# tud-amr/semantic_dsp_map

Hardware: AMD Instinct MI355X
Metric: Mvoxels updated/sec (256^3 grid, 2M particles, VKITTI2 camera; whole hot-path frame) (higher is better)
Workload: dtype f32

## Files before the change

### semantic_dsp_map_amd/csrc/kernels.hip

```cpp
#include <algorithm>

#include <type_traits>

#include <hip/hip_ext.h>
#include "sdm_internal.h"
#include "sdm_scratch.h"

#pragma clang fp contract(off)

namespace sdm {

namespace {

constexpr int TPB = 256;

#ifdef SDM_AB_TIMERS
}
__device__ unsigned long long g_dbg[6][8192 * 4];
namespace {
#define DBG_T() wall_clock64()
#define DBG_PUTK(k, i, v) do { if (blockIdx.x < 8192) g_dbg[k][blockIdx.x * 4 + (i)] = (unsigned long long)(v); } while (0)
#define DBG_PUT(i, v) DBG_PUTK(0, i, v)
#define DBG_LANE0(k, i) do { if (threadIdx.x == 0 && threadIdx.y == 0) DBG_PUTK(k, i, DBG_T()); } while (0)
#else
// ... 1659 lines not shown
  for (int j = 0; j < VIS_J; ++j) {
    if (code[j] == 0xffffffffu || flg[j]) continue;
    if (imz[j] <= imd[j]) {
      st.vts[lvv[j]] = (uint16_t)f.gts;
      mark_tile(st, lvv[j], f.epoch);
    }
  }
  __syncthreads();
  DBG_LANE0(1, 2);
  const uint32_t nf = n_full;
  for (uint32_t k = threadIdx.x; k < nf; k += TPB) {
    const uint32_t c = full_list[k];
    const uint32_t g = g0 + (c >> 6);
    const int ax = ((wlo + (int)(g % nwx)) << 6) + (int)(c & 63u);
    const int ay = f.bb0[1] + (int)((g / nwx) % by);
    const int az = f.bb0[2] + (int)(g / ((uint32_t)nwx * by));
    visibility_voxel<S>(d, f, st, sc, depth_img, ax, ay, az);
  }
  DBG_LANE0(1, 3);
  }
}

__device__ __forceinline__ void sift_down(uint32_t *a, uint32_t start, uint32_t end) {
  uint32_t root = start;
  while (2 * root + 1 <= end) {
    uint32_t child = 2 * root + 1, sw = root;
    if (a[sw] < a[child]) sw = child;
    if (child + 1 <= end && a[sw] < a[child + 1]) sw = child + 1;
    if (sw == root) return;
    uint32_t t = a[root];
    a[root] = a[sw];
    a[sw] = t;
    root = sw;
  }
}

constexpr int A7_ROWS = 16;
constexpr int A7_ITEMS = 16;
constexpr uint32_t CK_LIGHT_MAX = 4;
enum : uint8_t { CK_DONE = 0, CK_LIGHT = 1, CK_HEAVY = 2 };

__device__ __forceinline__ void ck_store(const Filter &flt, const Scratch &sc, float *__restrict__ ck_out, int finish, int p,
                                         const sdm_labeled_point &o, float ck) {
  if (finish) {
    const float ckk = ck * flt.p_detect + flt.noise_number;
    sc.ck_kappa[p] = ckk;
    sc.pix4[p] = make_float4(o.x, o.y, o.z, ckk);
    sc.pixt[p] = (uint32_t)o.track_id | (1u << 16);
  } else {
    ck_out[p] = ck;
  }
}

constexpr int BR_TPB = 640;
constexpr int BR_WAVES = BR_TPB / 64;
constexpr int BR_MAXW = 1 << ROW_COL_BITS;
template <int PPT>
__global__ __launch_bounds__(BR_TPB) __attribute__((amdgpu_waves_per_eu(PPT <= 4 ? 5 : 4, PPT <= 4 ? 5 : 4))) void k_bin_rows(Dims d, State st, Scratch sc) {
  static_assert(PPT == 2 || PPT == 4 || PPT * BR_TPB >= BR_MAXW, "eight pixels per thread cover the widest image");
  __shared__ uint32_t pre[BR_MAXW + 1];
  __shared__ uint32_t wave_tot[BR_WAVES];
  __shared__ uint32_t s_base;
  const int r = blockIdx.x;
  DBG_LANE0(2, 0);
  if (r == (int)gridDim.x - 1 && threadIdx.x < 64) alias_compact_wave(st);
  const bool overflow = sc.cnt->overflow != 0;
  const int lane = threadIdx.x & 63, wid = threadIdx.x >> 6;
  const int W = d.W;
  uint32_t c[PPT];
  const int j0 = PPT * (int)threadIdx.x;
#pragma unroll
  for (int u = 0; u < PPT; ++u) c[u] = (!overflow && j0 + u < W) ? sc.bin_count[r * W + j0 + u] : 0u;
  uint32_t sub_n = 0;
  if (threadIdx.x < ROW_SUBS && !overflow) {
    sub_n = sc.row_cnt[(size_t)(r * ROW_SUBS + threadIdx.x) * ROW_CNT_STRIDE];
    if (sub_n > sc.row_cap) sub_n = sc.row_cap;
  }
  uint32_t inc = 0;
#pragma unroll
  for (int u = 0; u < PPT; ++u) inc += c[u];
  const uint32_t mine = inc;
#pragma unroll
  for (int off = 1; off < 64; off <<= 1) {
    const uint32_t t = __shfl_up(inc, off, 64);
    if (lane >= off) inc += t;
  }
  if (lane == 63) wave_tot[wid] = inc;
  __syncthreads();
  uint32_t before = 0, total = 0;
#pragma unroll
  for (int w = 0; w < BR_WAVES; ++w) {
    if (w < wid) before += wave_tot[w];
    total += wave_tot[w];
  }
  {
    uint32_t run = before + inc - mine;
#pragma unroll
    for (int u = 0; u < PPT; ++u) {
      if (j0 + u < W) pre[j0 + u] = run;
      run += c[u];
    }
  }
  if (threadIdx.x == 0) {
    pre[W] = total;
    s_base = total ? atomicAdd(&sc.cnt->n_vis, total) : 0u;
    if (total && (s_base > sc.cap_vis || total > sc.cap_vis - s_base)) {
      sc.cnt->overflow = 1;
      pre[W] = 0;
    }
  }
  uint32_t sub_ex[ROW_SUBS + 1];
  {
    uint32_t run = 0;
#pragma unroll
    for (int k = 0; k < ROW_SUBS; ++k) {
      sub_ex[k] = run;
      run += (uint32_t)__shfl(sub_n, k, 64);
    }
    sub_ex[ROW_SUBS] = run;
  }
  __shared__ uint32_t s_sub[ROW_SUBS + 1];
  if (threadIdx.x == 0) {
#pragma unroll
    for (int k = 0; k <= ROW_SUBS; ++k) s_sub[k] = sub_ex[k];
  }
  __syncthreads();
  const uint32_t base = s_base;
  uint32_t *__restrict__ bs = sc.bin_start + (size_t)r * (W + 1);
  const bool row_over = total != 0 && pre[W] == 0;
  {
    const int h = d.window_half;
#pragma unroll
    for (int u = 0; u < PPT; ++u) {
      const int j = j0 + u;
      if (j < W) {
        const uint32_t n = row_over ? 0u : pre[j + h + 1 > W ? W : j + h + 1] - pre[j - h < 0 ? 0 : j - h];
        sc.row_win[r * W + j] = (uint8_t)(n > 255u ? 255u : n);
      }
    }
  }
  for (int j = threadIdx.x; j <= W; j += BR_TPB) bs[j] = row_over ? 0u : base + pre[j];
  if (total == 0 || row_over) {
    DBG_LANE0(2, 1);
    return;
  }
  const uint32_t n_row = s_sub[ROW_SUBS];
  for (uint32_t g = threadIdx.x; g < n_row; g += BR_TPB) {
    int sub = 0;
#pragma unroll
    for (int k = 1; k < ROW_SUBS; ++k) sub += s_sub[k] <= g ? 1 : 0;
    const uint2 e = sc.row_list[(size_t)(r * ROW_SUBS + sub) * sc.row_cap + (g - s_sub[sub])];
    sc.bin_idx[base + pre[e.y & (uint32_t)(BR_MAXW - 1)] + (e.y >> ROW_COL_BITS)] = e.x;
  }
  __syncthreads();
  const size_t slot_base = (size_t)d.v_begin << d.p_n;
#pragma unroll
  for (int u = 0; u < PPT; ++u) {
    const uint32_t n = c[u];
    if (!n) continue;
    const uint32_t p = (uint32_t)(r * W + j0 + u);
    const uint32_t s = base + pre[j0 + u];
    uint32_t *a = sc.bin_idx + s;
    auto small_bin = [&](auto kk) {
      constexpr int K = decltype(kk)::value;
      uint32_t v[K];
#pragma unroll
      for (int i = 0; i < K; ++i) v[i] = (uint32_t)i < n ? a[i] : 0xffffffffu;
#pragma unroll
      for (int pass = 0; pass < K; ++pass)
#pragma unroll
        for (int i = pass & 1; i + 1 < K; i += 2) {
          const uint32_t lo = v[i] < v[i + 1] ? v[i] : v[i + 1], hi = v[i] < v[i + 1] ? v[i + 1] : v[i];
          v[i] = lo;
          v[i + 1] = hi;
        }
#pragma unroll
      for (int i0 = 0; i0 < K; i0 += 8) {
        if ((uint32_t)i0 >= n) break;
        float4 q[8];
        float w8[8];
        uint16_t t8[8];
#pragma unroll
        for (int i = 0; i < 8; ++i)
          if ((uint32_t)(i0 + i) < n) {
            const size_t li = (size_t)v[i0 + i] - slot_base;
            q[i] = st.pos4[li];
            q[i].w = __uint_as_float((uint32_t)st.forget[li]);
            const SlotRef sr = slot_ref_li(st, d.p_n, li);
            w8[i] = sr.w();
            t8[i] = sr.track();
          }
#pragma unroll
        for (int i = 0; i < 8; ++i)
          if ((uint32_t)(i0 + i) < n) {
            if (n > 1) a[i0 + i] = v[i0 + i];
            sc.vp4[s + i0 + i] = make_float4(q[i].x, q[i].y, q[i].z, w8[i]);
            sc.vtf[s + i0 + i] = (uint32_t)t8[i] | ((__float_as_uint(q[i].w) & 0xffu) << 16);
            sc.vpix[s + i0 + i] = p;
          }
      }
    };
    if (n <= 8) {
      small_bin(std::integral_constant<int, 8>{});
      continue;
    }
    if (n <= 16) {
      small_bin(std::integral_constant<int, 16>{});
      continue;
    }
    if (n > 1) {
      if (n <= 32) {
        for (uint32_t i = 1; i < n; ++i) {
          uint32_t x = a[i];
          uint32_t j = i;
          while (j > 0 && a[j - 1] > x) {
            a[j] = a[j - 1];
            --j;
          }
          a[j] = x;
        }
      } else {
        for (int start = (int)(n - 2) / 2; start >= 0; --start) sift_down(a, (uint32_t)start, n - 1);
        for (uint32_t end = n - 1; end > 0; --end) {
          uint32_t t = a[end];
          a[end] = a[0];
          a[0] = t;
          sift_down(a, 0, end - 1);
        }
      }
    }
    for (uint32_t i = 0; i < n; ++i) {
      const size_t li = (size_t)a[i] - slot_base;
      const float4 q = st.pos4[li];
      const SlotRef sr = slot_ref_li(st, d.p_n, li);
      sc.vp4[s + i] = make_float4(q.x, q.y, q.z, sr.w());
      sc.vtf[s + i] = (uint32_t)sr.track() | ((uint32_t)st.forget[li] << 16);
      sc.vpix[s + i] = p;
    }
  }
  DBG_LANE0(2, 1);
}

__global__ __launch_bounds__(TPB) void k_ck_classify(Dims d, Filter flt, Scratch sc, float *__restrict__ ck_out, int finish) {
  const uint32_t p = blockIdx.x * blockDim.x + threadIdx.x;
  const int W = d.W, H = d.H, h = d.window_half;
  const bool in_image = p < (uint32_t)(W * H);
  const bool overflow = sc.cnt->overflow != 0;
  sdm_labeled_point o;
  o.is_valid = 0;
  uint32_t total = 0;
  if (in_image) {
    o = load_point(sc.fa->cloud, p);
    const int i = (int)p / W;
    uint32_t rw[A7_ROWS];
#pragma unroll
    for (int r = 0; r < A7_ROWS; ++r) {
      const int ni = i + r - h;
      const bool ok = r <= 2 * h && ni >= 0 && ni < H;
      rw[r] = sc.row_win[(int)p + (ok ? (r - h) * W : 0)];
    }
    __builtin_amdgcn_sched_barrier(0);
#pragma unroll
    for (int r = 0; r < A7_ROWS; ++r) {
      const int ni = i + r - h;
      total += (r <= 2 * h && ni >= 0 && ni < H) ? rw[r] : 0u;
    }
  }
  uint8_t cls = CK_DONE;
  if (in_image && o.is_valid && total != 0 && !overflow) cls = total <= CK_LIGHT_MAX ? CK_LIGHT : CK_HEAVY;
  const unsigned long long hm = __ballot(cls == CK_HEAVY);
  if (hm) {
    const uint32_t lane = threadIdx.x & 63u;
    const uint32_t shard = blockIdx.x & (VIS_SHARDS - 1);
    uint32_t base = 0;
    if (lane == 0) base = atomicAdd(&sc.cnt->shard[shard].heavy, (uint32_t)__popcll(hm));
    base = (uint32_t)__shfl((int)base, 0, 64);
    if (cls == CK_HEAVY) sc.ck_heavy[shard * sc.cap_heavy + base + (uint32_t)__popcll(hm & ((1ull << lane) - 1ull))] = p;
  }
  if (!in_image) return;
  if (!finish) {
    sc.pix4[p] = make_float4(o.x, o.y, o.z, 0.f);
    sc.pixt[p] = o.is_valid ? ((uint32_t)o.track_id | (1u << 16)) : 0u;
  }
  if (!o.is_valid) {
    if (finish) sc.pixt[p] = 0;
  } else if (cls == CK_DONE) {
    ck_store(flt, sc, ck_out, finish, (int)p, o, 0.f);
  }
  sc.ck_class[p] = cls;
}


template <bool FAST>
__device__ __forceinline__ float ck_term(const Filter &flt, const float *__restrict__ pdf, const float4 pv, const uint32_t tf,
                                         const sdm_labeled_point &o, float rsig, bool &skip) {
  const uint16_t ptrack = (uint16_t)(tf & 0xffffu);
  skip = flt.independent && ptrack != o.track_id;
  const float fg = flt.forget[(tf >> 16) & 7];
  float gk = query_pdf_r<FAST>(pdf, pv.x, o.x, o.sigma, rsig) * query_pdf_r<FAST>(pdf, pv.y, o.y, o.sigma, rsig) *
             query_pdf_r<FAST>(pdf, pv.z, o.z, o.sigma, rsig);
  if (!flt.independent) {
    gk *= fg;
    if (ptrack != o.track_id) gk *= flt.id_transition;
  }
  return pv.w * gk;
}

__device__ __forceinline__ void ck_light_pixel(const Dims &d, const Filter &flt, const State &st, const Scratch &sc,
                                               float *__restrict__ ck_out, int finish, int p) {
  const bool mine = p < d.W * d.H && sc.ck_class[p] == CK_LIGHT;
  sdm_labeled_point o;
  uint32_t ss[A7_ROWS], ee[A7_ROWS];
  if (mine) {
    o = load_point(sc.fa->cloud, p);
    const int h = d.window_half;
    const int i = p / d.W, j = p - i * d.W;
    const int j0 = j - h < 0 ? 0 : j - h;
    const int j1 = j + h >= d.W ? d.W - 1 : j + h;
#pragma unroll
    for (int r = 0; r < A7_ROWS; ++r) {
      const int ni = i + r - h;
      ss[r] = ee[r] = 0;
      if (r <= 2 * h && ni >= 0 && ni < d.H) {
        ss[r] = sc.bin_start[ni * (d.W + 1) + j0];
        ee[r] = sc.bin_start[ni * (d.W + 1) + j1 + 1];
      }
    }
  }
  float ck = 0.f;
  const float *__restrict__ pdf = st.pdf;
  const float rsig = mine ? div_recip(o.sigma) : 1.f;
  auto rows = [&](auto fast) {
#pragma unroll
    for (int r = 0; r < A7_ROWS; ++r) {
      if (ss[r] == ee[r]) continue;
      float acc = 0.f;
      for (uint32_t k = ss[r]; k < ee[r]; ++k) {
        bool skip;
        const float t = ck_term<decltype(fast)::value>(flt, pdf, sc.vp4[k], sc.vtf[k], o, rsig, skip);
        if (!skip) acc += t;
      }
      ck += acc;
    }
  };
  if (__ballot(rsig == 0.f) == 0ull) {
    if (mine) rows(std::true_type{});
  } else {
    if (mine) rows(std::false_type{});
  }
  if (mine) ck_store(flt, sc, ck_out, finish, p, o, ck);
}

#ifndef SDM_CK_TERM_CAP
#define SDM_CK_TERM_CAP 3584
#endif
constexpr uint32_t CK_TERM_CAP = SDM_CK_TERM_CAP;

#ifndef SDM_CK_HEAVY_PER_LIST
#define SDM_CK_HEAVY_PER_LIST 28
#endif
constexpr uint32_t CK_HEAVY_BLOCKS = SDM_CK_HEAVY_PER_LIST * VIS_SHARDS;
#ifndef SDM_CK_WAVES
#define SDM_CK_WAVES 7
#endif
#define CK_WAVES_ATTR __attribute__((amdgpu_waves_per_eu(SDM_CK_WAVES, SDM_CK_WAVES)))

__global__ __launch_bounds__(A7_ROWS *A7_ITEMS) CK_WAVES_ATTR void k_ck(Dims d, Filter flt, State st, Scratch sc,
                                                          float *__restrict__ ck_out, int finish) {
  DBG_LANE0(3, 0);
  if (blockIdx.x >= CK_HEAVY_BLOCKS) {
    ck_light_pixel(d, flt, st, sc, ck_out, finish,
                   (int)((blockIdx.x - CK_HEAVY_BLOCKS) * (A7_ROWS * A7_ITEMS) + threadIdx.y * A7_ROWS + threadIdx.x));
    DBG_LANE0(3, 1);
    return;
  }
  __shared__ float rowsum[A7_ITEMS][A7_ROWS];
  __shared__ uint32_t rowoff[A7_ITEMS * A7_ROWS + 1];
  __shared__ uint32_t rowbeg[A7_ITEMS * A7_ROWS];
  __shared__ float opx[A7_ITEMS][5];
  __shared__ uint32_t otrk[A7_ITEMS];
  __shared__ float term[CK_TERM_CAP];
  __shared__ uint8_t rowof[CK_TERM_CAP];
  const int r = threadIdx.x, it = threadIdx.y;
  const int lane = it * A7_ROWS + r;
  const int h = d.window_half;
  const uint32_t shard = blockIdx.x & (VIS_SHARDS - 1);
  const uint32_t n = sc.cnt->shard[shard].heavy;
  const float *__restrict__ pdf = st.pdf;
  const gptr<sdm_labeled_point> cloud_img = as_global(sc.fa->cloud);
  __shared__ uint32_t s_q0, s_slow;
  for (;;) {
    __syncthreads();
    if (lane == 0) {
      s_q0 = atomicAdd(&sc.cnt->shard[shard].heavy_ticket, (uint32_t)A7_ITEMS);
      s_slow = 0;
    }
    __syncthreads();
    const uint32_t q0 = s_q0;
    if (q0 >= n) break;
#ifdef SDM_AB_TIMERS
    if (lane == 0) g_dbg[3][blockIdx.x * 4 + 2] += 1;
#endif
    const uint32_t q = q0 + it;
    int p = 0;
    uint32_t s = 0, e = 0;
    sdm_labeled_point o;
    if (q < n) {
      p = (int)sc.ck_heavy[shard * sc.cap_heavy + q];
      o = load_point(sc.fa->cloud, p);
      const int i = p / d.W, j = p - i * d.W;
      const int ni = i + r - h;
      if (r <= 2 * h && ni >= 0 && ni < d.H) {
        const int j0 = j - h < 0 ? 0 : j - h;
        const int j1 = j + h >= d.W ? d.W - 1 : j + h;
        s = sc.bin_start[ni * (d.W + 1) + j0];
        e = sc.bin_start[ni * (d.W + 1) + j1 + 1];
      }
      if (r == 0) {
        opx[it][0] = o.x;
        opx[it][1] = o.y;
        opx[it][2] = o.z;
        opx[it][3] = o.sigma;
        opx[it][4] = div_recip(o.sigma);
        if (opx[it][4] == 0.f) s_slow = 1;
        otrk[it] = o.track_id;
// ... 1146 lines not shown
      SDM_DISPATCH_S(k_occupancy_scan_lists, sgrid, s, d, flt.occ_threshold, st, cnt, st.occ_need, grid.x, remark);
      SDM_DISPATCH_S(k_occupancy_listed, dim3(OCC_LISTED_GRID), s, d, flt.occ_threshold, st, remark);
    } else {
      SDM_DISPATCH_S(k_occupancy_scan, sgrid, s, d, flt.occ_threshold, st, cnt, st.occ_need, grid.x, remark);
    }
    SDM_DISPATCH_S(k_occupancy_dense, grid, s, d, flt.occ_threshold, st, cnt, st.occ_need, remark, grid.x);
  } else {
    const uint32_t n_tiles = grid.x;
    const uint32_t seg = n_tiles <= TPB * OCC_SEG_MAX ? ((n_tiles + TPB - 1) / TPB + 15u) / 16u * 16u : 0u;
    if (seg) grid = dim3(std::min<uint32_t>(OCC_GRID, n_tiles));
    SDM_DISPATCH_S(k_occupancy, grid, s, d, flt.occ_threshold, st, cnt, fa, n_tiles, seg);
  }
}


void launch_set_frame(FrameArgs *fa_dev, const FrameArgs &fa, hipStream_t s) {
  hipLaunchKernelGGL(k_set_frame, dim3(1), dim3(TPB), 0, s, fa_dev, fa);
}
const void *set_frame_kernel() { return reinterpret_cast<const void *>(k_set_frame); }

void launch_frustum(const Dims &d, const Scratch &sc, hipStream_t s) {
  static bool lds_attr_set = false;
  if (!lds_attr_set) {
    (void)hipFuncSetAttribute(reinterpret_cast<const void *>(k_flood2d), hipFuncAttributeMaxDynamicSharedMemorySize, 152 * 1024);
    lds_attr_set = true;
  }
  const size_t max_words = (size_t)(d.NY + 1) * (d.NZ + 1) * sc.wpl;
  const unsigned g_mask = (unsigned)std::min<size_t>(blocks_for(max_words * 64), 4096);
  const unsigned g_line = (unsigned)std::min<size_t>(blocks_for((size_t)sc.wy * (d.NZ + 1) * 64), 256);
  hipLaunchKernelGGL(k_vertex_mask, dim3(g_mask), dim3(TPB), 0, s, d, sc.fa_side, sc.vmask, sc.wpl, sc.cnt);
  hipLaunchKernelGGL(k_line_info, dim3(g_line), dim3(TPB), 0, s, d, sc.fa_side, sc.vmask, sc.wpl, sc.wy, sc.line_ne, sc.line_ey, sc.line_ez,
                     sc.cnt);
  hipLaunchKernelGGL(k_flood2d, dim3(1), dim3(TPB), (size_t)(d.NZ + 1) * sc.wy * 8 * 4, s, d, sc.fa_side, sc.vmask, sc.wpl, sc.wy, sc.line_ey,
                     sc.line_ez, sc.line_reach, sc.cnt);
  hipLaunchKernelGGL(k_flood_generic, dim3(1), dim3(1024), 0, s, d, sc.fa_side, sc.vmask, sc.reach, sc.wpl, sc.cnt);
}

void launch_visibility(const Dims &d, const Filter &flt, const State &st, const Scratch &sc, float *ck_out, int finish, hipStream_t s,
                       hipEvent_t vis_done) {
  {
    const size_t max_words = (size_t)((d.NX + 63) / 64 + 1) * d.NY * d.NZ;
    dim3 grid((unsigned)std::min<size_t>(blocks_for(max_words, VIS_WORDS), 2048));
    if (vis_done) {
      switch (d.p_n) {
        case 1: hipExtLaunchKernelGGL(k_visibility<2>, grid, dim3(TPB), 0, s, nullptr, vis_done, 0, d, st, sc); break;
        case 2: hipExtLaunchKernelGGL(k_visibility<4>, grid, dim3(TPB), 0, s, nullptr, vis_done, 0, d, st, sc); break;
        case 3: hipExtLaunchKernelGGL(k_visibility<8>, grid, dim3(TPB), 0, s, nullptr, vis_done, 0, d, st, sc); break;
        default: hipExtLaunchKernelGGL(k_visibility<16>, grid, dim3(TPB), 0, s, nullptr, vis_done, 0, d, st, sc); break;
      }
    } else {
      SDM_DISPATCH_S(k_visibility, grid, s, d, st, sc);
    }
  }
  if (d.W <= 2 * BR_TPB) hipLaunchKernelGGL(k_bin_rows<2>, dim3((unsigned)d.H), dim3(BR_TPB), 0, s, d, st, sc);
  else if (d.W <= 4 * BR_TPB) hipLaunchKernelGGL(k_bin_rows<4>, dim3((unsigned)d.H), dim3(BR_TPB), 0, s, d, st, sc);
  else hipLaunchKernelGGL(k_bin_rows<8>, dim3((unsigned)d.H), dim3(BR_TPB), 0, s, d, st, sc);
  hipLaunchKernelGGL(k_ck_classify, dim3(blocks_for((size_t)d.W * d.H)), dim3(TPB), 0, s, d, flt, sc, ck_out, finish);
}

void launch_ck(const Dims &d, const Filter &flt, const State &st, const Scratch &sc, float *ck_out, int finish, hipStream_t s) {
  hipLaunchKernelGGL(k_ck, dim3(CK_HEAVY_BLOCKS + blocks_for((size_t)d.W * d.H, A7_ROWS * A7_ITEMS)), dim3(A7_ROWS, A7_ITEMS), 0, s, d, flt, st, sc,
                     ck_out, finish);
}
void launch_ck_finish(const Dims &d, const Filter &flt, const Scratch &sc, const float *parts, int n_parts, size_t part_stride, hipStream_t s) {
  hipLaunchKernelGGL(k_ck_finish, dim3(blocks_for((size_t)d.W * d.H)), dim3(TPB), 0, s, d, flt, sc, parts, n_parts,
                     part_stride ? part_stride : (size_t)d.W * d.H);
}
void launch_ck_reduce_chunk(const float *stage, const float *own_part, float *full, uint32_t chunk, int world, int rank, hipStream_t s) {
  hipLaunchKernelGGL(k_ck_reduce_chunk, dim3((chunk + TPB - 1) / TPB), dim3(TPB), 0, s, stage, own_part, full, chunk, world, rank);
}
void launch_weight(const Dims &d, const Filter &flt, const State &st, const Scratch &sc, hipStream_t s, const float *ck_raw) {
  const int side = 2 * d.window_half + 1;
#define SDM_WEIGHT(UU, RR)                                                                                              \
  if (ck_raw) hipLaunchKernelGGL((k_weight<UU, RR, true>), dim3(WT_GRID), dim3(64 * WT_WAVES), 0, s, d, flt, st, sc, ck_raw); \
  else hipLaunchKernelGGL((k_weight<UU, RR, false>), dim3(WT_GRID), dim3(64 * WT_WAVES), 0, s, d, flt, st, sc, ck_raw);
  if (side * side <= 64) {
    SDM_WEIGHT(4, 1)
  } else if (side * side <= 128) {
    SDM_WEIGHT(4, 2)
  } else {
    SDM_WEIGHT(2, 4)
  }
#undef SDM_WEIGHT
}

int launch_birth_prepare(const Dims &d, const Filter &flt, const BirthOrder &bo, const State &st,
                         const Scratch &sc, hipStream_t s) {
  const size_t hw = (size_t)d.W * d.H;
  const size_t total = hw * flt.nb;
  if (flt.use_rng) {
    hipLaunchKernelGGL(k_birth_flags, dim3(blocks_for(hw)), dim3(TPB), 0, s, d, bo, sc);
    exclusive_scan_u32(sc.b_valid, sc.b_rank, hw, sc.scan_scratch_b, s);
  }
  hipLaunchKernelGGL(k_birth_candidates, dim3(blocks_for(total)), dim3(TPB), 0, s, d, flt, bo, st, sc);
  if (flt.use_rng) hipLaunchKernelGGL(k_birth_cursor, dim3(1), dim3(64), 0, s, d, flt, sc);
  int nbits = d.x_n + d.y_n + d.z_n + 1;
  return radix_sort_pairs(sc.bkey_a, sc.bval_a, sc.bkey_b, sc.bval_b, total, nbits, sc.sort_scratch, s);
}

void launch_birth_replay(const Dims &d, const Filter &flt, const State &st, const Scratch &sc, int which, bool literal,
                         hipStream_t s) {
  const size_t total = (size_t)d.W * d.H * flt.nb;
  const uint32_t *skey = which ? sc.bkey_b : sc.bkey_a;
  const uint32_t *sval = which ? sc.bval_b : sc.bval_a;
  dim3 grid(blocks_for(total));
#define SDM_BIRTH(SS)                                                                                                  \
  if (literal) hipLaunchKernelGGL((k_birth_replay<SS, true>), grid, dim3(TPB), 0, s, d, flt, st, sc, skey, sval, (uint32_t)total); \
  else hipLaunchKernelGGL((k_birth_replay<SS, false>), grid, dim3(TPB), 0, s, d, flt, st, sc, skey, sval, (uint32_t)total);
  switch (d.p_n) {
    case 1: SDM_BIRTH(2) break;
    case 2: SDM_BIRTH(4) break;
    case 3: SDM_BIRTH(8) break;
    default: SDM_BIRTH(16) break;
  }
#undef SDM_BIRTH
// ... 164 lines not shown
```

### semantic_dsp_map_amd/csrc/lifecycle.hip

```cpp
#include <rocrand/rocrand.h>

#include <chrono>
#include <cmath>
#include <cstdlib>
#include <mutex>

#include "sdm_map.h"

#pragma clang fp contract(off)

namespace {

thread_local std::string g_last_error;

__attribute__((constructor(101))) void sdm_runtime_defaults() {
  setenv("HIP_FORCE_DEV_KERNARG", "1", 0);
}

constexpr double GRAPH_PIECES_US = 110.0, GRAPH_CHAIN_US = 170.0;
constexpr int LAUNCHES_PER_FRAME = 50;

__global__ void k_noop() {}

}
// ... 390 lines not shown
  A(m->st.forget, n_slots);
  HIP_TRY(hipMemsetAsync(m->st.forget, 0, n_slots, m->stream));
  A(m->st.rec, rec_array_bytes(d.v_count, d.S));
  const size_t v_groups = ((size_t)d.v_count + 511) / 512 * 512;
  A(m->st.vts, v_groups + 64);
  A(m->st.vflag, v_groups + 64);
  m->st.tile_stride = (uint32_t)tile_mark_bytes(d);
  A(m->st.tile_dirty, 2 * (size_t)m->st.tile_stride);
  A(m->st.occ_need, ((size_t)d.v_count + 63) / 64 + 32);
  A(m->st.occ_list, occ_list_tiles(d.v_count) * OCC_LIST_CAP);
  A(m->st.occ_list_n, occ_list_tiles(d.v_count) + 64);
  m->st.occ_unit_cap = (uint32_t)((occ_list_tiles(d.v_count) + OCC_LIST_SHARDS - 1) / OCC_LIST_SHARDS * (OCC_LIST_CAP / OCC_LIST_UNIT));
  A(m->st.occ_unit, (size_t)OCC_LIST_SHARDS * m->st.occ_unit_cap);
  A(m->st.occ_shard, OCC_LIST_SHARDS + 1);
  HIP_TRY(hipMemsetAsync(m->st.occ_shard, 0, (OCC_LIST_SHARDS + 1) * sizeof(State::OccListShard), m->stream));
  A(m->st.grp_hint, grp_hint_bytes(d.v_count));
  HIP_TRY(hipMemsetAsync(m->st.grp_hint, 0, grp_hint_bytes(d.v_count), m->stream));
  A(m->st.owner, n_slots);
  A(m->st.owner_flag, owner_flag_bytes(n_slots));
  A(m->st.owner_flag2, owner_flag2_bytes(n_slots));
  A(m->st.alias, 2 + 2 * ALIAS_CAP);
  m->st.alias_cap = ALIAS_CAP;
  HIP_TRY(hipMemsetAsync(m->st.alias, 0, 8, m->stream));
  A(m->st.alias_filter, ALIAS_FILTER_WORDS);
  HIP_TRY(hipMemsetAsync(m->st.alias_filter, 0, ALIAS_FILTER_WORDS * 4, m->stream));
  A(m->st.res, d.v_count);
  A(m->st.stamps_x, d.NX);
  A(m->st.stamps_y, d.NY);
  A(m->st.stamps_z, d.NZ);
  A(m->st.pdf, PDF_NUM);
  m->noise_n = 1000000;
  A(m->st.noise, m->noise_n);
  HIP_TRY(hipMemsetAsync(m->st.noise, 0, (size_t)m->noise_n * 4, m->stream));
  {
    std::vector<float> pdf;
    build_pdf_table(pdf);
    HIP_TRY(hipMemcpyAsync(m->st.pdf, pdf.data(), PDF_NUM * 4, hipMemcpyHostToDevice, m->stream));
    HIP_TRY(hipStreamSynchronize(m->stream));
  }
  Scratch &sc = m->sc;
  sc.wpl = (int)((d.NX + 1 + 63) / 64);
  const size_t n_words = (size_t)(d.NZ + 1) * (d.NY + 1) * sc.wpl;
  A(sc.vmask, n_words);
  A(sc.reach, n_words);
  sc.wy = (int)((d.NY + 1 + 63) / 64);
  const size_t n_line_words = (size_t)(d.NZ + 1) * sc.wy;
  A(sc.line_ne, n_line_words);
  A(sc.line_ey, n_line_words);
  A(sc.line_ez, n_line_words);
  A(sc.line_reach, n_line_words);
  A(m->d_depth, hw);
  A(m->d_cloud, hw);
  A(sc.bin_count, hw + 1 + (size_t)d.H * ROW_SUBS * ROW_CNT_STRIDE);
  A(sc.row_win, hw);
  sc.row_cnt = sc.bin_count + hw + 1;
  A(sc.bin_start, (size_t)d.H * (d.W + 1));
  size_t cap_vis = cfg->max_visible > 0 ? (size_t)cfg->max_visible
                                        : std::min<size_t>(n_slots + (size_t)VIS_SHARDS * 256 * d.S, (size_t)16 << 20);
  cap_vis = (cap_vis + VIS_SHARDS - 1) / VIS_SHARDS * VIS_SHARDS;
  cap_vis = std::min<size_t>(cap_vis, 0xffffff00u);
  sc.cap_vis = (uint32_t)cap_vis;
  {
    const size_t row_total = std::min<size_t>(cap_vis, std::max<size_t>(2 * cap_vis / (size_t)d.H, (size_t)2 * d.W * d.S));
    sc.row_cap = (uint32_t)std::max<size_t>(64, (row_total + row_total / 4) / ROW_SUBS + 64);
  }
  A(sc.row_list, (size_t)d.H * ROW_SUBS * sc.row_cap);
  A(sc.bin_idx, cap_vis);
  A(sc.vpix, cap_vis);
  A(sc.vp4, cap_vis);
  A(sc.vtf, cap_vis);
  A(sc.pix4, hw);
  A(sc.pixt, hw);
  A(sc.ck_kappa, hw);
  sc.cap_heavy = (uint32_t)(((hw + 255) / 256 + VIS_SHARDS - 1) / VIS_SHARDS * 256);
  A(sc.ck_heavy, (size_t)sc.cap_heavy * VIS_SHARDS);
  A(sc.ck_class, hw);
  m->ck_chunk = (uint32_t)(((hw + shard_count - 1) / shard_count + 63) / 64 * 64);
  A(m->d_ck_part, (size_t)m->ck_chunk * shard_count);
  for (auto &r : m->raw) {
    A(r.depth, hw);
    A(r.static_mask, hw);
    A(r.label_to_inst, 256);
    A(r.bbox, 6 * MAX_CLOUD_OBJECTS);
  }
  A(sc.b_valid, hw + 1);
  A(sc.b_rank, hw + 1);
  sc.cap_move = (uint32_t)std::min<size_t>((size_t)d.V * d.S, (size_t)1 << 18);
  A(m->d_counts_local, HALO_OBJ);
  const size_t mv_cnt_n = move_count_elems();
  A(sc.mv_cnt, mv_cnt_n);
  A(sc.mv_list, 8192);
  A(sc.mv_nlist, 4);
  HIP_TRY(hipMemsetAsync(sc.mv_nlist, 0, 4 * sizeof(uint32_t), m->stream));
  A(sc.mv_nmem, 8192);
  A(sc.mv_mem, move_member_elems(n_slots));
  A(sc.mv_tot, move_total_elems());
  HIP_TRY(hipMemsetAsync(sc.mv_tot, 0, move_total_elems() * sizeof(uint32_t), m->stream));
  A(m->d_track_bits, 2048);
  A(sc.mv_copy, sc.cap_move);
  A(sc.track_to_obj, 65536);
  HIP_TRY(hipMemsetAsync(sc.track_to_obj, 0xFF, 65536, m->stream));
  size_t scan_need = scan_scratch_elems(hw + 1);
  A(sc.scan_scratch, scan_need + 16);
  A(sc.scan_scratch_b, scan_scratch_elems(hw + 1) + 16);
  HIP_TRY(hipMemsetAsync(sc.scan_scratch, 0, (scan_need + 16) * 4, m->stream));
  HIP_TRY(hipMemsetAsync(sc.scan_scratch_b, 0, (scan_scratch_elems(hw + 1) + 16) * 4, m->stream));
  A(sc.mv_row, (size_t)d.v_count * MV_ROW);
  HIP_TRY(hipMemsetAsync(sc.mv_row, 0xff, (size_t)d.v_count * MV_ROW * sizeof(uint32_t), m->stream));
  A(sc.mv_next, sc.cap_move);
  A(sc.cnt, 1);
  A(sc.cur, 1);
  HIP_TRY(hipMemsetAsync(sc.cnt, 0, sizeof(Counters), m->stream));
  HIP_TRY(hipMemsetAsync(sc.cur, 0, sizeof(Cursors), m->stream));
  A(m->d_fa[0], 1);
  A(m->d_fa[1], 1);
  A(m->d_fa[2], 1);
  for (FrameArgs *p : m->d_fa) HIP_TRY(hipMemsetAsync(p, 0, sizeof(FrameArgs), m->stream));
  m->sc.fa = m->d_fa[0];
  m->sc.fa_side = m->d_fa[1];
  m->sc.fa_moves = m->d_fa[2];
  A(m->d_u64, 1);
  A(m->emit.mask, emit_mask_bytes(d));
  A(m->emit.blk_cnt, emit_block_elems(d));
  A(m->emit.total, 4);
#undef A
  m->cur_depth = m->d_depth;
  m->cur_cloud = m->d_cloud;
  {
    const char *e = getenv("SDM_GRAPH");
// ... 181 lines not shown
```

### semantic_dsp_map_amd/csrc/sdm_internal.h

```cpp
#pragma once
#include <hip/hip_runtime.h>
#include <stdint.h>

#include "../../include/sdm.h"

#pragma clang fp contract(off)

namespace sdm {

constexpr uint32_t INVALID_INDEX = 0xffffffffu;
constexpr uint16_t OWNER_NONE = 0xFFFF;
constexpr int PDF_NUM = 20000;
#define SDM_OCC_INIT_WEIGHT 0.05f
#define SDM_MIN_RIGHT_PDF 0.1f

enum : uint8_t { ST_INVALID = 0, ST_UPDATED = 1, ST_REGULAR_BORN = 2, ST_GUESSED_BORN = 3, ST_COPIED = 4, ST_TIMEPTC = 5 };

struct Dims {
  int x_n, y_n, z_n, p_n;
  uint32_t NX, NY, NZ, S;
  uint32_t V;
  uint32_t v_begin;
  uint32_t v_count;
  uint32_t rz_begin, rz_count;
// ... 4 lines not shown
  float dmin, dmax;
  float tanx, tany;
  float occl_coeff;
  int window_half;
  int max_movable;
};

struct Frame {
  int eq[3];
  float center[3];
  uint32_t gts;
  uint32_t epoch;
  float E[16];
  int bb0[3], bb1[3];
  int start_v[3];
  int start_ok;
};

struct Filter {
  float p_detect, noise_number, occ_threshold, id_transition;
  float forget[8];
  int independent;
  int consider_depth_noise;
  int nb;
  int use_rng;
  int noise_n;
};

struct Counters {
  uint32_t n_vis;
  uint32_t n_birth_success;
  uint32_t n_birth_attempts;
  uint32_t n_resampled;
  uint32_t n_moved;
  uint32_t n_move_reinserted;
  uint32_t n_frustum_voxels;
  uint32_t n_occupied;
  uint32_t n_free;
  uint32_t overflow;
  uint32_t n_valid_px;
  uint32_t n_halo_dropped;
  uint32_t vis_flood_complex, vis_flood_rounds, vis_start_in_frustum;
  uint32_t n_moved_b[2];
  uint32_t pad[2];
  struct alignas(128) ShardLine {
    uint32_t vis;
    uint32_t fv;
    uint32_t heavy;
    uint32_t birth;
    uint32_t resample;
    uint32_t sweep;
    uint32_t sweep_tiles;
    uint32_t heavy_ticket;
    uint32_t pad[24];
  };
  ShardLine shard[64];
  uint32_t flood_complex;
  uint32_t flood_rounds;
  uint32_t start_in_frustum;
  uint32_t flood_pad[29];
};
static_assert(sizeof(Counters::ShardLine) == 128, "one cache line per shard");
constexpr uint32_t VIS_SHARDS = 64;
constexpr uint32_t ROW_SUBS = 8;
constexpr int ROW_COL_BITS = 12, ROW_PIB_BITS = 32 - ROW_COL_BITS;
constexpr uint32_t ROW_CNT_STRIDE = 32;
constexpr uint32_t OWNER_CHUNK = 4096;
constexpr uint32_t OWNER_GROUP = 64;
__host__ __device__ constexpr size_t owner_flag_bytes(size_t n_slots) {
  return ((n_slots + OWNER_CHUNK - 1) / OWNER_CHUNK + OWNER_GROUP - 1) / OWNER_GROUP * OWNER_GROUP;
}
__host__ __device__ constexpr size_t owner_flag2_bytes(size_t n_slots) { return (owner_flag_bytes(n_slots) / OWNER_GROUP + 4095) / 4096 * 4096; }
constexpr int MAX_STAMP_UPDATES = 96;
struct StampUpdates {
  int n;
  uint32_t value;
  uint16_t entry[MAX_STAMP_UPDATES];
};
struct Cursors {
  int32_t birth_cursor;
  int32_t move_cursor;
  uint32_t move_list_overflow;
};

constexpr size_t REC_BYTES_PER_SLOT = 10;
__host__ __device__ constexpr uint32_t rec_bytes(uint32_t S) { return (uint32_t)REC_BYTES_PER_SLOT * (S - 1u); }
__host__ __device__ constexpr size_t rec_array_bytes(size_t v_count, uint32_t S) { return (v_count + 64) * rec_bytes(S) + 64; }
typedef float rec_f32 __attribute__((aligned(2)));
typedef uint32_t rec_v4u __attribute__((ext_vector_type(4), aligned(2)));
typedef uint32_t rec_v2u __attribute__((ext_vector_type(2), aligned(2)));

struct SlotRef {
  unsigned char *r;
  uint32_t L, k;
  __host__ __device__ __forceinline__ float w() const { return *reinterpret_cast<const rec_f32 *>(r + 4u * k); }
  __host__ __device__ __forceinline__ uint16_t ts() const { return *reinterpret_cast<const uint16_t *>(r + 4u * L + 2u * k); }
  __host__ __device__ __forceinline__ uint16_t track() const { return *reinterpret_cast<const uint16_t *>(r + 6u * L + 2u * k); }
  __host__ __device__ __forceinline__ uint8_t label() const { return r[8u * L + k]; }
  __host__ __device__ __forceinline__ uint8_t status() const { return r[9u * L + k]; }
  __host__ __device__ __forceinline__ void set_w(float v) const { *reinterpret_cast<rec_f32 *>(r + 4u * k) = v; }
  __host__ __device__ __forceinline__ void set_ts(uint16_t v) const { *reinterpret_cast<uint16_t *>(r + 4u * L + 2u * k) = v; }
  __host__ __device__ __forceinline__ void set_track(uint16_t v) const { *reinterpret_cast<uint16_t *>(r + 6u * L + 2u * k) = v; }
  __host__ __device__ __forceinline__ void set_label(uint8_t v) const { r[8u * L + k] = v; }
  __host__ __device__ __forceinline__ void set_status(uint8_t v) const { r[9u * L + k] = v; }
};

struct State {
  float4 *pos4 = nullptr;
  uint8_t *forget = nullptr;
  unsigned char *rec = nullptr;
  uint16_t *vts = nullptr;
  uint8_t *vflag = nullptr;
  uint8_t *tile_dirty = nullptr;
  uint32_t tile_stride = 0;
  unsigned long long *occ_need = nullptr;
  uint16_t *occ_list = nullptr;
  uint32_t *occ_list_n = nullptr;
  uint2 *occ_unit = nullptr;
  uint32_t occ_unit_cap = 0;
// ... 353 lines not shown
```

### semantic_dsp_map_amd/csrc/sdm_scratch.h

```cpp
#pragma once
#include "sdm_internal.h"

namespace sdm {

struct BirthOrder {
  int off[10];
  int cols[9];
};

struct MoveCopy {
  float x, y, z;
  uint32_t forget_bits;
  float w;
  uint16_t ts, track, owner;
  uint8_t label, status;
  uint32_t voxel;
};
static_assert(sizeof(MoveCopy) == 32, "MoveCopy layout");

constexpr int MAX_MOVE_OBJECTS = 48;
constexpr int MAX_REMOVE_TRACKS = 128;
constexpr int HALO_OBJ = 64;
constexpr int HALO_RECORD_BYTES = 36;
constexpr int HALO_HEADER_BYTES = 16;
__host__ __device__ constexpr size_t halo_segment_bytes(uint32_t cap) { return HALO_HEADER_BYTES + (size_t)cap * HALO_RECORD_BYTES; }
struct MoveSet {
  int n;
  float T[MAX_MOVE_OBJECTS][12];
  uint16_t track[MAX_MOVE_OBJECTS];
};

struct FrameArgs {
  Frame f;
  StampUpdates su;
  MoveSet ms;
  int n_obj;
  int n_remove;
  uint32_t mv_seq;
  uint32_t mv_batch;
  int force_generic;
  const float *depth;
  const sdm_labeled_point *cloud;
  uint16_t remove[MAX_REMOVE_TRACKS];
};
static_assert(sizeof(FrameArgs) <= 3400, "FrameArgs travels as a kernel argument (4 KB limit, with the launch's other arguments)");

constexpr int MV_ROW = 16;
constexpr int MV_DIRECT = MV_ROW - 2;
constexpr uint32_t MV_FIRST = 0x100u;
struct Scratch {
  const FrameArgs *fa = nullptr;
  const FrameArgs *fa_side = nullptr;
  const FrameArgs *fa_moves = nullptr;
  uint64_t *vmask = nullptr, *reach = nullptr;
  int wpl = 0;
  uint64_t *line_ne = nullptr, *line_ey = nullptr, *line_ez = nullptr, *line_reach = nullptr;
  int wy = 0;
  uint32_t *bin_count = nullptr, *bin_start = nullptr;
  uint32_t *row_cnt = nullptr;
  uint8_t *row_win = nullptr;
  uint2 *row_list = nullptr;
  uint32_t row_cap = 0;
  uint32_t cap_vis = 0;
  uint32_t *bin_idx = nullptr, *vpix = nullptr;
  float4 *vp4 = nullptr;
  uint32_t *vtf = nullptr;
  float4 *pix4 = nullptr;
  uint32_t *pixt = nullptr;
  float *ck_kappa = nullptr;
  uint8_t *ck_class = nullptr;
  uint32_t *ck_heavy = nullptr;
  uint32_t cap_heavy = 0;
  uint32_t *b_valid = nullptr, *b_rank = nullptr;
  uint32_t *bkey_a = nullptr, *bval_a = nullptr, *bkey_b = nullptr, *bval_b = nullptr;
  float4 *bpos = nullptr;
  uint32_t *mv_cnt = nullptr;
  uint32_t *mv_list = nullptr, *mv_nlist = nullptr;
  uint32_t *mv_nmem = nullptr, *mv_mem = nullptr, *mv_tot = nullptr;
  MoveCopy *mv_copy = nullptr;
  uint32_t cap_move = 0;
  unsigned char *halo_send = nullptr;
  const unsigned char *halo_recv = nullptr;
  uint32_t halo_cap = 0;
  uint32_t halo_world = 1;
  uint8_t *track_to_obj = nullptr;
  uint32_t *scan_scratch = nullptr, *sort_scratch = nullptr;
  uint32_t *scan_scratch_b = nullptr;
  uint32_t *mv_row = nullptr, *mv_next = nullptr;
  Counters *cnt = nullptr;
  Cursors *cur = nullptr;
};

constexpr int MAX_CLOUD_OBJECTS = 64;
struct CloudArgsHost {
  double R[9], t[3];
  double ifx, icx, ify, icy;
  double dmin, dmax;
  float sigma0, sigma1;
  int consider_depth_noise, consider_instance, n_objects, has_static;
  int sky_instance, has_bbox;
  int track[MAX_CLOUD_OBJECTS], label[MAX_CLOUD_OBJECTS];
};
void launch_labeled_cloud(const Dims &d, const CloudArgsHost &h, const float *depth, const uint8_t *static_mask,
                          const uint16_t *label_to_inst, const uint8_t *obj_masks, const double *bbox,
                          sdm_labeled_point *cloud, hipStream_t s);
void launch_manual_resize(const Dims &d, const void *src, void *dst, int src_w, int src_h, float scale, int elem_bytes,
                          hipStream_t s);

void launch_set_frame(FrameArgs *fa_dev, const FrameArgs &fa, hipStream_t s);
const void *set_frame_kernel();
struct MembersArgs {
  uint32_t *mv_cnt, *mv_list, *mv_nlist, *mv_nmem, *mv_mem, *mv_tot;
  Cursors *cur;
  uint32_t n_flags;
  size_t n_slots;
};
struct FrameBeginLaunch {
#ifndef SDM_FB_GRID
#define SDM_FB_GRID 1024
#endif
  static constexpr unsigned GRID = SDM_FB_GRID, BLOCK = 256;
  Counters *cnt;
  uint32_t *bin_count;
  uint32_t n_bins;
// ... 71 lines not shown
```

Before: 95850.

## Fuse pixel classification into row binning and compact light pixels into lists

Moves the per-pixel light/heavy classification, previously its own kernel reading a row_win byte plane, into k_bin_rows. That kernel now reads bin_count over the vertical window, forms column sums in shared memory and sums them horizontally. Light pixels are now compacted into sharded lists like heavy ones, so the ck kernel launches a fixed grid that walks those lists instead of one block per image tile checking a class byte. This removes a kernel launch, the row_win and ck_class buffers and idle light blocks. In exchange k_bin_rows does more loads and register work per thread, and the output order of the lists changes.

```diff
diff --git a/semantic_dsp_map_amd/csrc/kernels.hip b/semantic_dsp_map_amd/csrc/kernels.hip
--- a/semantic_dsp_map_amd/csrc/kernels.hip
+++ b/semantic_dsp_map_amd/csrc/kernels.hip
@@ -1735,30 +1735,66 @@
   }
 }
 
-constexpr int BR_TPB = 640;
-constexpr int BR_WAVES = BR_TPB / 64;
 constexpr int BR_MAXW = 1 << ROW_COL_BITS;
 template <int PPT>
-__global__ __launch_bounds__(BR_TPB) __attribute__((amdgpu_waves_per_eu(PPT <= 4 ? 5 : 4, PPT <= 4 ? 5 : 4))) void k_bin_rows(Dims d, State st, Scratch sc) {
+__global__ __launch_bounds__(BR_TPB) __attribute__((amdgpu_waves_per_eu(PPT <= 4 ? 5 : 4, PPT <= 4 ? 5 : 4))) void k_bin_rows(
+    Dims d, Filter flt, State st, Scratch sc, float *__restrict__ ck_out, int finish) {
   static_assert(PPT == 2 || PPT == 4 || PPT * BR_TPB >= BR_MAXW, "eight pixels per thread cover the widest image");
   __shared__ uint32_t pre[BR_MAXW + 1];
+  __shared__ uint32_t colsum[BR_MAXW];
   __shared__ uint32_t wave_tot[BR_WAVES];
   __shared__ uint32_t s_base;
   const int r = blockIdx.x;
   DBG_LANE0(2, 0);
   if (r == (int)gridDim.x - 1 && threadIdx.x < 64) alias_compact_wave(st);
-  const bool overflow = sc.cnt->overflow != 0;
   const int lane = threadIdx.x & 63, wid = threadIdx.x >> 6;
-  const int W = d.W;
+  const int W = d.W, H = d.H, h = d.window_half;
+  const sdm_labeled_point *cloud = sc.fa->cloud;
+  const uint32_t ovf = sc.cnt->overflow;
   uint32_t c[PPT];
   const int j0 = PPT * (int)threadIdx.x;
-#pragma unroll
-  for (int u = 0; u < PPT; ++u) c[u] = (!overflow && j0 + u < W) ? sc.bin_count[r * W + j0 + u] : 0u;
-  uint32_t sub_n = 0;
-  if (threadIdx.x < ROW_SUBS && !overflow) {
-    sub_n = sc.row_cnt[(size_t)(r * ROW_SUBS + threadIdx.x) * ROW_CNT_STRIDE];
-    if (sub_n > sc.row_cap) sub_n = sc.row_cap;
-  }
+  int jc[PPT];
+#pragma unroll
+  for (int u = 0; u < PPT; ++u) jc[u] = j0 + u < W ? j0 + u : W - 1;
+#pragma unroll
+  for (int u = 0; u < PPT; ++u) c[u] = sc.bin_count[r * W + jc[u]];
+  uint32_t sub_n = sc.row_cnt[(size_t)(r * ROW_SUBS + (threadIdx.x < ROW_SUBS ? threadIdx.x : ROW_SUBS - 1)) * ROW_CNT_STRIDE];
+  constexpr int PH = PPT <= 4 ? PPT : 4;
+  sdm_labeled_point o_first[PH];
+#pragma unroll
+  for (int u0 = 0; u0 < PPT; u0 += 2) {
+    uint32_t nb[A7_ROWS][2];
+#pragma unroll
+    for (int k = 0; k < A7_ROWS; ++k) {
+      const int ni = r + k - h;
+      const bool ok = k <= 2 * h && ni >= 0 && ni < H;
+      const uint32_t *__restrict__ row = sc.bin_count + (ok ? ni : r) * W;
+      nb[k][0] = row[jc[u0]];
+      nb[k][1] = row[jc[u0 + 1]];
+    }
+    __builtin_amdgcn_sched_barrier(0);
+    if constexpr (PPT <= 4) {
+      if (u0 == 0) {
+#pragma unroll
+        for (int u = 0; u < PH; ++u) o_first[u] = load_point(cloud, (size_t)(r * W + jc[u]));
+        __builtin_amdgcn_sched_barrier(0);
+      }
+    }
+    uint32_t s0 = 0, s1 = 0;
+#pragma unroll
+    for (int k = 0; k < A7_ROWS; ++k) {
+      const int ni = r + k - h;
+      const bool ok = k <= 2 * h && ni >= 0 && ni < H;
+      s0 += ok ? nb[k][0] : 0u;
+      s1 += ok ? nb[k][1] : 0u;
+    }
+    if (j0 + u0 < W) colsum[j0 + u0] = s0;
+    if (j0 + u0 + 1 < W) colsum[j0 + u0 + 1] = s1;
+  }
+  const bool overflow = ovf != 0;
+#pragma unroll
+  for (int u = 0; u < PPT; ++u) c[u] = (!overflow && j0 + u < W) ? c[u] : 0u;
+  sub_n = (overflow || threadIdx.x >= ROW_SUBS) ? 0u : (sub_n > sc.row_cap ? sc.row_cap : sub_n);
   uint32_t inc = 0;
 #pragma unroll
   for (int u = 0; u < PPT; ++u) inc += c[u];
@@ -1770,6 +1806,57 @@
   }
   if (lane == 63) wave_tot[wid] = inc;
   __syncthreads();
+  uint32_t cls = 0, list_base = 0;
+  {
+    uint32_t n_heavy = 0, n_light = 0;
+#pragma unroll
+    for (int v0 = 0; v0 < PPT; v0 += PH) {
+      sdm_labeled_point o[PH];
+      if constexpr (PPT <= 4) {
+#pragma unroll
+        for (int u = 0; u < PH; ++u) o[u] = o_first[u];
+      } else {
+#pragma unroll
+        for (int u = 0; u < PH; ++u) o[u] = load_point(cloud, (size_t)(r * W + jc[v0 + u]));
+      }
+      uint32_t cs[A7_ROWS - 1 + PH];
+#pragma unroll
+      for (int k = 0; k < A7_ROWS - 1 + PH; ++k) {
+        const int j = j0 + v0 - h + k;
+        const bool ok = k <= 2 * h + PH - 1 && j >= 0 && j < W;
+        cs[k] = colsum[ok ? j : 0];
+        cs[k] = ok ? cs[k] : 0u;
+      }
+#pragma unroll
+      for (int u = 0; u < PH; ++u) {
+        uint32_t wtot = 0;
+#pragma unroll
+        for (int k = u; k < A7_ROWS - 1 + PH; ++k) wtot += k <= u + 2 * h ? cs[k] : 0u;
+        const int j = j0 + v0 + u;
+        const bool in_image = j < W;
+        const bool valid = in_image && o[u].is_valid;
+        uint32_t cl = CK_DONE;
+        if (valid && wtot != 0 && !overflow) cl = wtot <= CK_LIGHT_MAX ? CK_LIGHT : CK_HEAVY;
+        cls |= cl << (2 * (v0 + u));
+        n_heavy += (uint32_t)__popcll(__ballot(cl == CK_HEAVY));
+        n_light += (uint32_t)__popcll(__ballot(cl == CK_LIGHT));
+        if (!in_image) continue;
+        const int p = r * W + j;
+        if (!finish) {
+          sc.pix4[p] = make_float4(o[u].x, o[u].y, o[u].z, 0.f);
+          sc.pixt[p] = o[u].is_valid ? ((uint32_t)o[u].track_id | (1u << 16)) : 0u;
+        }
+        if (!o[u].is_valid) {
+          if (finish) sc.pixt[p] = 0;
+        } else if (cl == CK_DONE) {
+          ck_store(flt, sc, ck_out, finish, p, o[u], 0.f);
+        }
+      }
+    }
+    Counters::ShardLine &line = sc.cnt->shard[ck_list_shard(r, wid)];
+    const uint32_t n_mine = lane == 0 ? n_heavy : n_light;
+    if (lane < 2 && n_mine) list_base = atomicAdd(lane == 0 ? &line.heavy : &line.light, n_mine);
+  }
   uint32_t before = 0, total = 0;
 #pragma unroll
   for (int w = 0; w < BR_WAVES; ++w) {
@@ -1811,15 +1898,18 @@
   const uint32_t base = s_base;
   uint32_t *__restrict__ bs = sc.bin_start + (size_t)r * (W + 1);
   const bool row_over = total != 0 && pre[W] == 0;
-  {
-    const int h = d.window_half;
+  if (__ballot(cls != 0) != 0ull) {
+    const uint32_t first = ck_list_shard(r, wid) * sc.cap_heavy;
+    uint32_t at_h = first + (uint32_t)__shfl((int)list_base, 0, 64), at_l = first + (uint32_t)__shfl((int)list_base, 1, 64);
+    const unsigned long long below = (1ull << lane) - 1ull;
 #pragma unroll
     for (int u = 0; u < PPT; ++u) {
-      const int j = j0 + u;
-      if (j < W) {
-        const uint32_t n = row_over ? 0u : pre[j + h + 1 > W ? W : j + h + 1] - pre[j - h < 0 ? 0 : j - h];
-        sc.row_win[r * W + j] = (uint8_t)(n > 255u ? 255u : n);
-      }
+      const uint32_t cl = (cls >> (2 * u)) & 3u;
+      const unsigned long long hm = __ballot(cl == CK_HEAVY), lm = __ballot(cl == CK_LIGHT);
+      if (cl == CK_HEAVY) sc.ck_heavy[at_h + (uint32_t)__popcll(hm & below)] = (uint32_t)(r * W + j0 + u);
+      if (cl == CK_LIGHT) sc.ck_light[at_l + (uint32_t)__popcll(lm & below)] = (uint32_t)(r * W + j0 + u);
+      at_h += (uint32_t)__popcll(hm);
+      at_l += (uint32_t)__popcll(lm);
     }
   }
   for (int j = threadIdx.x; j <= W; j += BR_TPB) bs[j] = row_over ? 0u : base + pre[j];
@@ -1924,55 +2014,6 @@
   DBG_LANE0(2, 1);
 }
 
-__global__ __launch_bounds__(TPB) void k_ck_classify(Dims d, Filter flt, Scratch sc, float *__restrict__ ck_out, int finish) {
-  const uint32_t p = blockIdx.x * blockDim.x + threadIdx.x;
-  const int W = d.W, H = d.H, h = d.window_half;
-  const bool in_image = p < (uint32_t)(W * H);
-  const bool overflow = sc.cnt->overflow != 0;
-  sdm_labeled_point o;
-  o.is_valid = 0;
-  uint32_t total = 0;
-  if (in_image) {
-    o = load_point(sc.fa->cloud, p);
-    const int i = (int)p / W;
-    uint32_t rw[A7_ROWS];
-#pragma unroll
-    for (int r = 0; r < A7_ROWS; ++r) {
-      const int ni = i + r - h;
-      const bool ok = r <= 2 * h && ni >= 0 && ni < H;
-      rw[r] = sc.row_win[(int)p + (ok ? (r - h) * W : 0)];
-    }
-    __builtin_amdgcn_sched_barrier(0);
-#pragma unroll
-    for (int r = 0; r < A7_ROWS; ++r) {
-      const int ni = i + r - h;
-      total += (r <= 2 * h && ni >= 0 && ni < H) ? rw[r] : 0u;
-    }
-  }
-  uint8_t cls = CK_DONE;
-  if (in_image && o.is_valid && total != 0 && !overflow) cls = total <= CK_LIGHT_MAX ? CK_LIGHT : CK_HEAVY;
-  const unsigned long long hm = __ballot(cls == CK_HEAVY);
-  if (hm) {
-    const uint32_t lane = threadIdx.x & 63u;
-    const uint32_t shard = blockIdx.x & (VIS_SHARDS - 1);
-    uint32_t base = 0;
-    if (lane == 0) base = atomicAdd(&sc.cnt->shard[shard].heavy, (uint32_t)__popcll(hm));
-    base = (uint32_t)__shfl((int)base, 0, 64);
-    if (cls == CK_HEAVY) sc.ck_heavy[shard * sc.cap_heavy + base + (uint32_t)__popcll(hm & ((1ull << lane) - 1ull))] = p;
-  }
-  if (!in_image) return;
-  if (!finish) {
-    sc.pix4[p] = make_float4(o.x, o.y, o.z, 0.f);
-    sc.pixt[p] = o.is_valid ? ((uint32_t)o.track_id | (1u << 16)) : 0u;
-  }
-  if (!o.is_valid) {
-    if (finish) sc.pixt[p] = 0;
-  } else if (cls == CK_DONE) {
-    ck_store(flt, sc, ck_out, finish, (int)p, o, 0.f);
-  }
-  sc.ck_class[p] = cls;
-}
-
 
 template <bool FAST>
 __device__ __forceinline__ float ck_term(const Filter &flt, const float *__restrict__ pdf, const float4 pv, const uint32_t tf,
@@ -1990,8 +2031,7 @@
 }
 
 __device__ __forceinline__ void ck_light_pixel(const Dims &d, const Filter &flt, const State &st, const Scratch &sc,
-                                               float *__restrict__ ck_out, int finish, int p) {
-  const bool mine = p < d.W * d.H && sc.ck_class[p] == CK_LIGHT;
+                                               float *__restrict__ ck_out, int finish, int p, bool mine) {
   sdm_labeled_point o;
   uint32_t ss[A7_ROWS], ee[A7_ROWS];
   if (mine) {
@@ -2043,6 +2083,10 @@
 #define SDM_CK_HEAVY_PER_LIST 28
 #endif
 constexpr uint32_t CK_HEAVY_BLOCKS = SDM_CK_HEAVY_PER_LIST * VIS_SHARDS;
+#ifndef SDM_CK_LIGHT_PER_LIST
+#define SDM_CK_LIGHT_PER_LIST 8
+#endif
+constexpr uint32_t CK_LIGHT_BLOCKS = SDM_CK_LIGHT_PER_LIST * VIS_SHARDS;
 #ifndef SDM_CK_WAVES
 #define SDM_CK_WAVES 7
 #endif
@@ -2051,9 +2095,16 @@
 __global__ __launch_bounds__(A7_ROWS *A7_ITEMS) CK_WAVES_ATTR void k_ck(Dims d, Filter flt, State st, Scratch sc,
                                                           float *__restrict__ ck_out, int finish) {
   DBG_LANE0(3, 0);
-  if (blockIdx.x >= CK_HEAVY_BLOCKS) {
-    ck_light_pixel(d, flt, st, sc, ck_out, finish,
-                   (int)((blockIdx.x - CK_HEAVY_BLOCKS) * (A7_ROWS * A7_ITEMS) + threadIdx.y * A7_ROWS + threadIdx.x));
+  if (blockIdx.x < CK_LIGHT_BLOCKS) {
+    const uint32_t shard = blockIdx.x & (VIS_SHARDS - 1);
+    const uint32_t n = sc.cnt->shard[shard].light;
+    constexpr uint32_t WG = A7_ROWS * A7_ITEMS;
+    for (uint32_t q0 = (blockIdx.x / VIS_SHARDS) * WG; q0 < n; q0 += SDM_CK_LIGHT_PER_LIST * WG) {
+      const uint32_t q = q0 + threadIdx.y * A7_ROWS + threadIdx.x;
+      const bool mine = q < n;
+      const int p = mine ? (int)sc.ck_light[shard * sc.cap_heavy + q] : 0;
+      ck_light_pixel(d, flt, st, sc, ck_out, finish, p, mine);
+    }
     DBG_LANE0(3, 1);
     return;
   }
@@ -3306,15 +3357,15 @@
       SDM_DISPATCH_S(k_visibility, grid, s, d, st, sc);
     }
   }
-  if (d.W <= 2 * BR_TPB) hipLaunchKernelGGL(k_bin_rows<2>, dim3((unsigned)d.H), dim3(BR_TPB), 0, s, d, st, sc);
-  else if (d.W <= 4 * BR_TPB) hipLaunchKernelGGL(k_bin_rows<4>, dim3((unsigned)d.H), dim3(BR_TPB), 0, s, d, st, sc);
-  else hipLaunchKernelGGL(k_bin_rows<8>, dim3((unsigned)d.H), dim3(BR_TPB), 0, s, d, st, sc);
-  hipLaunchKernelGGL(k_ck_classify, dim3(blocks_for((size_t)d.W * d.H)), dim3(TPB), 0, s, d, flt, sc, ck_out, finish);
+  switch (br_ppt(d.W)) {
+    case 2: hipLaunchKernelGGL(k_bin_rows<2>, dim3((unsigned)d.H), dim3(BR_TPB), 0, s, d, flt, st, sc, ck_out, finish); break;
+    case 4: hipLaunchKernelGGL(k_bin_rows<4>, dim3((unsigned)d.H), dim3(BR_TPB), 0, s, d, flt, st, sc, ck_out, finish); break;
+    default: hipLaunchKernelGGL(k_bin_rows<8>, dim3((unsigned)d.H), dim3(BR_TPB), 0, s, d, flt, st, sc, ck_out, finish); break;
+  }
 }
 
 void launch_ck(const Dims &d, const Filter &flt, const State &st, const Scratch &sc, float *ck_out, int finish, hipStream_t s) {
-  hipLaunchKernelGGL(k_ck, dim3(CK_HEAVY_BLOCKS + blocks_for((size_t)d.W * d.H, A7_ROWS * A7_ITEMS)), dim3(A7_ROWS, A7_ITEMS), 0, s, d, flt, st, sc,
-                     ck_out, finish);
+  hipLaunchKernelGGL(k_ck, dim3(CK_LIGHT_BLOCKS + CK_HEAVY_BLOCKS), dim3(A7_ROWS, A7_ITEMS), 0, s, d, flt, st, sc, ck_out, finish);
 }
 void launch_ck_finish(const Dims &d, const Filter &flt, const Scratch &sc, const float *parts, int n_parts, size_t part_stride, hipStream_t s) {
   hipLaunchKernelGGL(k_ck_finish, dim3(blocks_for((size_t)d.W * d.H)), dim3(TPB), 0, s, d, flt, sc, parts, n_parts,
diff --git a/semantic_dsp_map_amd/csrc/lifecycle.hip b/semantic_dsp_map_amd/csrc/lifecycle.hip
--- a/semantic_dsp_map_amd/csrc/lifecycle.hip
+++ b/semantic_dsp_map_amd/csrc/lifecycle.hip
@@ -466,7 +466,6 @@
   A(m->d_depth, hw);
   A(m->d_cloud, hw);
   A(sc.bin_count, hw + 1 + (size_t)d.H * ROW_SUBS * ROW_CNT_STRIDE);
-  A(sc.row_win, hw);
   sc.row_cnt = sc.bin_count + hw + 1;
   A(sc.bin_start, (size_t)d.H * (d.W + 1));
   size_t cap_vis = cfg->max_visible > 0 ? (size_t)cfg->max_visible
@@ -486,9 +485,9 @@
   A(sc.pix4, hw);
   A(sc.pixt, hw);
   A(sc.ck_kappa, hw);
-  sc.cap_heavy = (uint32_t)(((hw + 255) / 256 + VIS_SHARDS - 1) / VIS_SHARDS * 256);
+  sc.cap_heavy = ck_list_cap(d.W, d.H);
   A(sc.ck_heavy, (size_t)sc.cap_heavy * VIS_SHARDS);
-  A(sc.ck_class, hw);
+  A(sc.ck_light, (size_t)sc.cap_heavy * VIS_SHARDS);
   m->ck_chunk = (uint32_t)(((hw + shard_count - 1) / shard_count + 63) / 64 * 64);
   A(m->d_ck_part, (size_t)m->ck_chunk * shard_count);
   for (auto &r : m->raw) {
diff --git a/semantic_dsp_map_amd/csrc/sdm_internal.h b/semantic_dsp_map_amd/csrc/sdm_internal.h
--- a/semantic_dsp_map_amd/csrc/sdm_internal.h
+++ b/semantic_dsp_map_amd/csrc/sdm_internal.h
@@ -80,7 +80,8 @@
     uint32_t sweep;
     uint32_t sweep_tiles;
     uint32_t heavy_ticket;
-    uint32_t pad[24];
+    uint32_t light;
+    uint32_t pad[23];
   };
   ShardLine shard[64];
   uint32_t flood_complex;
@@ -93,6 +94,18 @@
 constexpr uint32_t ROW_SUBS = 8;
 constexpr int ROW_COL_BITS = 12, ROW_PIB_BITS = 32 - ROW_COL_BITS;
 constexpr uint32_t ROW_CNT_STRIDE = 32;
+constexpr int BR_TPB = 640;
+constexpr int BR_WAVES = BR_TPB / 64;
+__host__ __device__ constexpr int br_ppt(int W) { return W <= 2 * BR_TPB ? 2 : (W <= 4 * BR_TPB ? 4 : 8); }
+__host__ __device__ constexpr uint32_t ck_list_shard(int row, int wave) { return (uint32_t)(row * BR_WAVES + wave) & (VIS_SHARDS - 1); }
+inline uint32_t ck_list_cap(int W, int H) {
+  const int per_wave = 64 * br_ppt(W);
+  uint32_t n[VIS_SHARDS] = {}, cap = 0;
+  for (int r = 0; r < H; ++r)
+    for (int w = 0; w < BR_WAVES && w * per_wave < W; ++w) n[ck_list_shard(r, w)] += (uint32_t)(W - w * per_wave < per_wave ? W - w * per_wave : per_wave);
+  for (uint32_t k = 0; k < VIS_SHARDS; ++k) cap = n[k] > cap ? n[k] : cap;
+  return cap;
+}
 constexpr uint32_t OWNER_CHUNK = 4096;
 constexpr uint32_t OWNER_GROUP = 64;
 __host__ __device__ constexpr size_t owner_flag_bytes(size_t n_slots) {
diff --git a/semantic_dsp_map_amd/csrc/sdm_scratch.h b/semantic_dsp_map_amd/csrc/sdm_scratch.h
--- a/semantic_dsp_map_amd/csrc/sdm_scratch.h
+++ b/semantic_dsp_map_amd/csrc/sdm_scratch.h
@@ -58,7 +58,6 @@
   int wy = 0;
   uint32_t *bin_count = nullptr, *bin_start = nullptr;
   uint32_t *row_cnt = nullptr;
-  uint8_t *row_win = nullptr;
   uint2 *row_list = nullptr;
   uint32_t row_cap = 0;
   uint32_t cap_vis = 0;
@@ -68,8 +67,8 @@
   float4 *pix4 = nullptr;
   uint32_t *pixt = nullptr;
   float *ck_kappa = nullptr;
-  uint8_t *ck_class = nullptr;
   uint32_t *ck_heavy = nullptr;
+  uint32_t *ck_light = nullptr;
   uint32_t cap_heavy = 0;
   uint32_t *b_valid = nullptr, *b_rank = nullptr;
   uint32_t *bkey_a = nullptr, *bval_a = nullptr, *bkey_b = nullptr, *bval_b = nullptr;
```

Result: no change. 96290, median of 6 (+0.5%).
